# PlantandFoodResearch/MCHap

Measured on AMD Instinct MI355X. Metric: loci/sec (whole node) for 1000-step MCMC, tetraploid 8-SNV loci, 1/2/4/8 GPUs, higher is better.
Workload: dtype f64; 1 GPU; 10000 synthetic tetraploid loci per GPU, 8 SNVs, 200 reads, 1000 MCMC steps x 2 chains, burn 500, posterior summary (BASELINE.json configs[1]); 4 passes in flight on separate HIP streams, each with its own device buffers; loci_per_gpu=10000, ploidy=4, snvs=8, reads=200, mcmc_steps=1000, chains=2, burn=500, llk_cache=True, passes_in_flight=4, hw_queues=4, world_size=1, devices=1

## Files before the change

mchap_amd/csrc/denovo_kernel.hpp:

```cpp
#pragma once
#include <hip/hip_runtime.h>
#include <math.h>
#include <stdint.h>

#include "../../include/mchap_hip.h"
#include "philox.hpp"

namespace mchap {

constexpr int WAVE = 64;
constexpr uint32_t SLOT_INIT = 0xFFFFu;

static __constant__ double c_ln[260];
static __constant__ double c_ln_inv[260];

struct DenovoParams {
  const mchap_unit *units;
  const double *reads;
  const int64_t *counts;
  const int8_t *n_alleles;
  const int8_t *initial;
  uint64_t *trace;
  double *llks;
  int8_t *fixed;
// ... 42 lines not shown
  if (nb < M + 4) nb = M + 4;
  L.buf = o; o += 8 * nb;
  L.optin = o; o += 4 * K * K;
  L.sub = o; o += align8(2 * K * M);
  L.hetrow = o; o += align8(2 * M);
  L.shift = o; o += align8(M);
  L.nal = o; o += align8(M);
  L.total = align8(o);
  return L;
}

__host__ __device__ inline int allele_bits(int A) { return A <= 2 ? 1 : (A <= 4 ? 2 : 3); }

template <int CTRL>
__device__ __forceinline__ double wave_dpp_f64(double v) {
  const long long b = __double_as_longlong(v);
  const int lo = __builtin_amdgcn_update_dpp(0, (int)(unsigned)b, CTRL, 0xf, 0xf, false);
  const int hi = __builtin_amdgcn_update_dpp(0, (int)(unsigned)((unsigned long long)b >> 32), CTRL, 0xf, 0xf, false);
  return __longlong_as_double((long long)(((unsigned long long)(unsigned)hi << 32) | (unsigned)lo));
}
__device__ __forceinline__ double wave_sum(double v) {
#ifdef MCHAP_PLAIN_BUTTERFLY
#pragma unroll
  for (int o = 32; o >= 1; o >>= 1) v += __shfl_xor(v, o, WAVE);
#else
  v += __shfl_xor(v, 32, WAVE);
  v += __shfl_xor(v, 16, WAVE);
  v += wave_dpp_f64<0x128>(v);
  v += wave_dpp_f64<0x124>(v);
  v += wave_dpp_f64<0x122>(v);
  v += wave_dpp_f64<0x121>(v);
#endif
  return v;
}
static __global__ void wave_sum_kernel(const double *x, double *out) {
  const double s = wave_sum(x[(size_t)blockIdx.x * WAVE + threadIdx.x]);
  const bool same = __ballot(__double_as_longlong(s) == __double_as_longlong(__shfl(s, 0, WAVE))) == ~0ull;
  if (threadIdx.x == 0) out[blockIdx.x] = same ? s : __longlong_as_double(0x7ff8dead00000000ll);
}
__device__ __forceinline__ int wave_sum_i(int v) {
#pragma unroll
  for (int o = 32; o >= 1; o >>= 1) v += __shfl_xor(v, o, WAVE);
  return v;
}

__device__ __forceinline__ uint32_t nib(uint32_t p, int h) { return (p >> (4 * h)) & 15u; }
__device__ __forceinline__ uint32_t nib_set(uint32_t p, int h, uint32_t v) {
  return (p & ~(15u << (4 * h))) | (v << (4 * h));
}
__device__ __forceinline__ uint32_t nib(uint64_t p, int h) { return (uint32_t)(p >> (4 * h)) & 15u; }
__device__ __forceinline__ uint64_t nib_set(uint64_t p, int h, uint32_t v) {
  return (p & ~(15ull << (4 * h))) | ((uint64_t)v << (4 * h));
}

__device__ __forceinline__ double add_log_prob(double x, double y) {
  if (x == -INFINITY && y == -INFINITY) return -INFINITY;
  if (x > y) return x + log1p(exp(y - x));
  return y + log1p(exp(x - y));
}

__device__ __forceinline__ int choose_from(const double *p, int n, double u) {
  double c = 0.0;
  for (int i = 0; i < n; i++) {
    c += p[i];
    if (c > u) return i;
  }
// ... 783 lines not shown
```

mchap_amd/csrc/denovo_spec_kernel.hpp:

```cpp
#pragma once
#include <type_traits>

#include "denovo_simt_kernel.hpp"

#ifdef MCHAP_MASK_PADDING
#define MCHAP_PAD_LANE(x) (x)
#else
#define MCHAP_PAD_LANE(x) true
#endif
#ifndef MCHAP_COOP_UNR
#define MCHAP_COOP_UNR 2
#endif
#ifndef MCHAP_SPEC_TB
#define MCHAP_SPEC_TB 4
#endif
#ifndef MCHAP_SPEC_LOW
#define MCHAP_SPEC_LOW 8
#endif
#ifndef MCHAP_SPEC_CG
#define MCHAP_SPEC_CG 4
#endif
#ifndef MCHAP_SPEC_VAR
#define MCHAP_SPEC_VAR 0
#endif
#define MCHAP_SPEC_SBS (MCHAP_SPEC_VAR == 1)
#define MCHAP_SPEC_DEEP (MCHAP_SPEC_VAR == 2)
#ifndef MCHAP_SPEC_WIN0
#define MCHAP_SPEC_WIN0 4
#endif
#ifndef MCHAP_SPEC_WIN_MIN
#define MCHAP_SPEC_WIN_MIN 2
#endif
#ifndef MCHAP_REUSE_MAXK
#define MCHAP_REUSE_MAXK 8
#endif
#ifndef MCHAP_CODED_UNR
#define MCHAP_CODED_UNR 16
#endif

namespace mchap {

constexpr int SPEC_MAX_IV = 64;
constexpr int SPEC_TB = MCHAP_SPEC_TB;
constexpr int SPEC_LN = 72;
constexpr int SPEC_DRAWS_MAX = 384;
__host__ __device__ inline int spec_draws(int K, int Mmax) {
  int d = 2 * K * Mmax - 1;
  if (d < 3 * Mmax + 2) d = 3 * Mmax + 2;
  d = (d + 1) & ~1;
  return d < SPEC_DRAWS_MAX ? d : SPEC_DRAWS_MAX;
}

#define LDSP(T) __attribute__((address_space(3))) T *
#define GLBP(T) __attribute__((address_space(1))) T *
template <class T>
__device__ __forceinline__ LDSP(T) lds_cast(void *p) {
  return (LDSP(T))p;
}

// ... 26 lines not shown
  LDSP(double) optp;
  LDSP(double) optl;
  LDSP(double) ln;
  LDSP(double) lninv;
  LDSP(uint32_t) ivse;
  LDSP(uint32_t) ivlin;
  LDSP(uint32_t) ivlout;
  LDSP(uint32_t) ivno;
  LDSP(uint16_t) cols;
  LDSP(uint16_t) permtab;
  LDSP(uint8_t) shift;
  LDSP(uint8_t) nal;
  LDSP(uint8_t) ktab;
  LDSP(uint8_t) ordtab;
  LDSP(uint16_t) nreads;
  LDSP(uint16_t) ndict;
  LDSP(double) dict;
  LDSP(uint64_t) gptr;
  LDSP(double) gval;
  LDSP(uint32_t) gstream;
  LDSP(uint64_t) bw;
  LDSP(double) bpc;
  LDSP(uint64_t) bpt;
  LDSP(uint64_t) gbt;
  LDSP(const uint8_t) sct;
  LDSP(uint64_t) tbuf;
  LDSP(uint64_t) lc;
  uint32_t lc_mask;
  uint32_t cache_mask;
  int key_words;
  bool cache_on;
  uint64_t epoch = 0ull;
  bool reuse_on;
  bool cut_off = false;
  LDSP(const uint8_t) lds_ct;
  LDSP(const double) lds_cw;
  int crow;
  LDSP(uint64_t) draws;
  LDSP(double) memo_tot;
  LDSP(double) bdist;
  int memo_stride;
  int ndraws;
  LDSP(unsigned char) cx_lds;
  LDSP(double) cx_val;
  uint64_t *cx_base = nullptr;
  int cx_n = 0;
};

__host__ __device__ inline int spec_memo_entries(int Mmax) { return Mmax * (Mmax + 1) / 2; }
__host__ __device__ inline int spec_memo_index(int start, int stop) { return stop * (stop - 1) / 2 + start; }
__host__ __device__ inline size_t spec_memo_bytes(int Mmax, int T, int G) {
  const size_t per_group = (size_t)2 * spec_memo_entries(Mmax) * 8;
  if (T != 1 || per_group > 16 * 1024) return 0;
  return per_group * (64 / G);
}

constexpr int SPEC_LC_ENTRIES = 256;
#ifndef MCHAP_LC_GEN
#define MCHAP_LC_GEN 48
#endif
constexpr uint32_t SPEC_LC_SECOND_LEVEL_GEN = MCHAP_LC_GEN;
__host__ __device__ inline size_t spec_lc_bytes(int entries = SPEC_LC_ENTRIES) { return (size_t)16 * entries + 16; }
__host__ __device__ inline bool spec_ctx_in_bpc(int K, int Mmax, int Amax, int max_reads) {
  return K >= 3 && max_reads <= 64 && Mmax * Amax <= 24 * (K - 2) && 16 * K * Mmax <= 3 * 64 * 8 && 12 * 64 + 4 * 8 <= 3 * 64 * 8;
}
__host__ __device__ inline int spec_lc_entries(int bp_cache) { return (bp_cache & 2) ? ((bp_cache & 4) ? SPEC_LC_ENTRIES / 2 : SPEC_LC_ENTRIES) : 0; }
// ... 536 lines not shown
__device__ __forceinline__ void spec_hap_prod(LDSP(double) dict, const PairRows rows, int p0, int Mh, typename TabPtr<LT>::u8 ct,
                                              int crow, double (&prod)[RPL]) {
  constexpr int UNR = 8;
  constexpr int GB = 2;
#pragma unroll
  for (int i = 0; i < RPL; i++) prod[i] = 1.0;
  for (int j0 = 0; j0 < Mh; j0 += UNR) {
    CT cd[UNR];
#pragma unroll
    for (int u = 0; u < UNR; u++) {
      const int p = __builtin_amdgcn_readfirstlane(p0 + min(j0 + u, Mh - 1));
      const int row = p < WAVE ? __builtin_amdgcn_readlane(rows.r0, p & (WAVE - 1))
                               : (p < 2 * WAVE ? __builtin_amdgcn_readlane(rows.r1, p & (WAVE - 1)) : __builtin_amdgcn_readlane(rows.r2, p & (WAVE - 1)));
      cd[u] = TabPtr<LT>::template ld<CT>(ct + (size_t)row * crow);
    }
#pragma unroll
    for (int u0 = 0; u0 < UNR; u0 += GB) {
      if (j0 + u0 < Mh) {
        double f[GB][RPL];
#pragma unroll
        for (int u = 0; u < GB; u++)
#pragma unroll
          for (int i = 0; i < RPL; i++) f[u][i] = dict[((uint32_t)cd[u0 + u] >> (8 * i)) & 255u];
#pragma unroll
        for (int u = 0; u < GB; u++) {
          const bool on = j0 + u0 + u < Mh;
#pragma unroll
          for (int i = 0; i < RPL; i++) prod[i] *= on ? f[u][i] : 1.0;
        }
      }
    }
  }
}
template <int KT, bool IN_LDS>
struct BaseProducts;
template <int KT>
struct BaseProducts<KT, false> {
  double v[KT][4];
  __device__ __forceinline__ double get(int h, int i, int) const { return v[h][i]; }
  __device__ __forceinline__ void set(int h, int i, int, double x) { v[h][i] = x; }
};
template <int KT>
struct BaseProducts<KT, true> {
  LDSP(double) p;
  __device__ __forceinline__ double get(int h, int i, int lane) const { return p[(h * 4 + i) * WAVE + lane]; }
  __device__ __forceinline__ void set(int h, int i, int lane, double x) { p[(h * 4 + i) * WAVE + lane] = x; }
};
template <int KT>
struct BaseProductsG {
  GLBP(double) p;
  int rpad, cb;
  __device__ __forceinline__ double get(int h, int i, int lane) const { return p[(size_t)h * rpad + (cb + i) * WAVE + lane]; }
  __device__ __forceinline__ void set(int h, int i, int lane, double x) { p[(size_t)h * rpad + (cb + i) * WAVE + lane] = x; }
};
template <int KT, int RPL, class CT, bool LT = false, class BP>
__device__ __forceinline__ double spec_coop_reuse(const SpecLds &S, int src, int sg, int mmax, int Mh, uint32_t amask,
                                                  typename TabPtr<LT>::u8 ct, typename TabPtr<LT>::f64 cw, int crow, int lane,
                                                  const BP &bp, bool use_base, bool grouped) {
  LDSP(double) dict = S.dict + (size_t)sg * DICT_MAX;
  const double invK = 1.0 / (double)KT;
  const PairRows rows = spec_pair_rows<KT>(S.pw, WAVE, src, S, sg, mmax, Mh, amask, lane);
  double acc[RPL];
#pragma unroll
  for (int i = 0; i < RPL; i++) acc[i] = 0.0;
#pragma unroll
  for (int h = 0; h < KT; h++) {
    const uint64_t a = S.pw[(size_t)h * WAVE + src], b = S.bw[(size_t)sg * KT + h];
    const bool same = use_base && __builtin_amdgcn_readfirstlane((int)(a == b)) != 0;
    double ph[RPL];
    if (same) {
#pragma unroll
      for (int i = 0; i < RPL; i++) ph[i] = bp.get(h, i, lane);
    } else {
      spec_hap_prod<RPL, CT, LT>(dict, rows, h * Mh, Mh, ct, crow, ph);
    }
#pragma unroll
    for (int i = 0; i < RPL; i++) acc[i] += ph[i] * invK;
  }
  double wv[RPL];
#pragma unroll
  for (int i = 0; i < RPL; i++) wv[i] = cw[WAVE * i];
  return read_log_sum<RPL>(acc, wv, grouped);
}
template <int KT, int RPL, class CT, bool LT = false>
__device__ __forceinline__ double spec_coop_reuse_g(const SpecLds &S, int src, int sg, int mmax, int Mh, uint32_t amask,
                                                    typename TabPtr<LT>::u8 ct, typename TabPtr<LT>::f64 cw, int crow, int lane,
                                                    const BaseProductsG<KT> &bg, bool grouped) {
  double bpv[KT][RPL];
#pragma unroll
  for (int h = 0; h < KT; h++)
#pragma unroll
    for (int i = 0; i < RPL; i++) bpv[h][i] = bg.get(h, i, lane);
  LDSP(double) dict = S.dict + (size_t)sg * DICT_MAX;
  const double invK = 1.0 / (double)KT;
  const PairRows rows = spec_pair_rows<KT>(S.pw, WAVE, src, S, sg, mmax, Mh, amask, lane);
  double acc[RPL];
#pragma unroll
  for (int i = 0; i < RPL; i++) acc[i] = 0.0;
#pragma unroll
  for (int h = 0; h < KT; h++) {
    const uint64_t a = S.pw[(size_t)h * WAVE + src], b = S.bw[(size_t)sg * KT + h];
    const bool same = __builtin_amdgcn_readfirstlane((int)(a == b)) != 0;
    double ph[RPL];
    if (same) {
#pragma unroll
      for (int i = 0; i < RPL; i++) ph[i] = bpv[h][i];
    } else {
      spec_hap_prod<RPL, CT, LT>(dict, rows, h * Mh, Mh, ct, crow, ph);
    }
#pragma unroll
    for (int i = 0; i < RPL; i++) acc[i] += ph[i] * invK;
  }
  double wv[RPL];
#pragma unroll
  for (int i = 0; i < RPL; i++) wv[i] = cw[WAVE * i];
  return read_log_sum<RPL>(acc, wv, grouped);
}
template <int KT, int RPL, class CT, bool LT = false, class BP>
__device__ __forceinline__ void spec_base_products(const SpecLds &S, int sg, int mmax, int Mh, uint32_t amask,
                                                   typename TabPtr<LT>::u8 ct, int crow, int lane, BP &bp) {
  LDSP(double) dict = S.dict + (size_t)sg * DICT_MAX;
  const PairRows rows = spec_pair_rows<KT>(S.bw + (size_t)sg * KT, 1, 0, S, sg, mmax, Mh, amask, lane);
#pragma unroll
  for (int h = 0; h < KT; h++) {
    double ph[RPL];
    spec_hap_prod<RPL, CT, LT>(dict, rows, h * Mh, Mh, ct, crow, ph);
#pragma unroll
    for (int i = 0; i < RPL; i++) bp.set(h, i, lane, ph[i]);
  }
}
template <int KT, int RPL, class CT, bool LT = false, class BP>
__device__ __forceinline__ void spec_base_products_of(const SpecLds &S, const PairRows rows, int sg, int h, int Mh,
                                                      typename TabPtr<LT>::u8 ct, int crow, int lane, BP &bp) {
  LDSP(double) dict = S.dict + (size_t)sg * DICT_MAX;
  double ph[RPL];
  spec_hap_prod<RPL, CT, LT>(dict, rows, h * Mh, Mh, ct, crow, ph);
#pragma unroll
  for (int i = 0; i < RPL; i++) bp.set(h, i, lane, ph[i]);
}

template <int KT>
__device__ __forceinline__ unsigned long long spec_same_request(LDSP(uint64_t) pwbuf, unsigned long long reqs, int src, int lane) {
  if ((reqs & (reqs - 1ull)) == 0ull) return reqs;
  bool eq = ((reqs >> lane) & 1ull) != 0ull;
#pragma unroll
  for (int h = 0; h < KT; h++) eq = eq & (pwbuf[(size_t)h * WAVE + lane] == pwbuf[(size_t)h * WAVE + src]);
  return __ballot(eq);
}

template <int KT, int G, bool LT = false, bool DEDUP = true>
__device__ __forceinline__ double spec_coop_all(unsigned long long todo, LDSP(uint64_t) pwbuf, LDSP(uint8_t) shift_tab,
                                                LDSP(uint16_t) cols_tab, LDSP(uint16_t) nreads_tab, LDSP(uint16_t) ndict_tab,
                                                LDSP(double) dict_tab, LDSP(uint64_t) gptr_tab, LDSP(uint64_t) bw_tab,
                                                bool reuse, int crow, int mmax, int Mh_lane, uint32_t amask_lane, int rpad,
                                                int lane, LDSP(const uint8_t) lds_ct = nullptr, LDSP(const double) lds_cw = nullptr,
                                                LDSP(double) bpc = nullptr, LDSP(uint64_t) bpt = nullptr,
                                                LDSP(const uint8_t) sct = nullptr, LDSP(uint64_t) gbt = nullptr) {
  SpecLds S;
  S.pw = pwbuf;
  S.shift = shift_tab;
  S.cols = cols_tab;
  S.dict = dict_tab;
  S.bw = bw_tab;
  const int nch_batch = rpad / WAVE;
  double val = 0.0;
  while (todo) {
    const int sg = (__ffsll((long long)todo) - 1) / G;
    const unsigned long long gmask = G == 64 ? ~0ull : (((1ull << (G & 63)) - 1ull) << (sg * (G & 63)));
    unsigned long long reqs = todo & gmask;
    todo &= ~gmask;
    const int first = __ffsll((long long)reqs) - 1;
    const int Mh = __builtin_amdgcn_readfirstlane(__shfl(Mh_lane, first, WAVE));
    const uint32_t amask = (uint32_t)__builtin_amdgcn_readfirstlane(__shfl((int)amask_lane, first, WAVE));
    LDSP(uint64_t) gp = gptr_tab + sg * GP_N;
    GLBP(const double) rt = (GLBP(const double))(uintptr_t)gp[GP_RT] + lane;
    typename TabPtr<LT>::f64 cw;
    if constexpr (LT) cw = lds_cw + lane;
    else cw = (GLBP(const double))(uintptr_t)gp[GP_CW] + lane;
    const int nrd = (int)nreads_tab[sg];
    const bool grouped = nd_w01(ndict_tab[sg]);
    const int nch = max(1, min(nch_batch, (nrd + WAVE - 1) / WAVE));
    const int cstride = crow / WAVE;
    if (MCHAP_REUSE_MAXK >= KT && nd_count(ndict_tab[sg]) != 0 && KT * Mh <= (MCHAP_SPEC_DEEP ? 3 : 2) * WAVE) {
      const int nb0 = nch < 4 ? nch : 4;
      typename TabPtr<LT>::u8 ct;
      if constexpr (LT) ct = lds_ct + (size_t)lane * cstride;
      else ct = (GLBP(const uint8_t))(uintptr_t)gp[GP_CT] + (size_t)lane * cstride;
      constexpr bool BPL = (G == 64) && !LT;
      bool cached = false;
      if (BPL && bpc != nullptr) {
// ... 303 lines not shown
              double acc[4] = {0.0, 0.0, 0.0, 0.0};
#pragma unroll
              for (int h = 0; h < KT; h++) {
                const uint64_t wa = pwbuf[(size_t)h * WAVE + my_src], wb = bw_tab[(size_t)sg * KT + h];
                double ph[4];
                if (wa == wb) {
#pragma unroll
                  for (int k = 0; k < 4; k++) ph[k] = k < RK ? bpc[(h * 4) * WAVE + r + 16 * k] : 0.0;
                } else {
                  hap_products(wa, ph);
                }
#pragma unroll
                for (int k = 0; k < 4; k++) acc[k] += ph[k] * invK;
              }
#pragma unroll
              for (int k = 0; k < 4; k++)
                if (k < RK) v[k] = read_log(acc[k]) * cwr[k];
            }
            const double a0 = RK > 2 ? v[0] + v[2] : v[0];
            const double a1 = RK > 3 ? v[1] + v[3] : v[1];
            double sv = RK > 1 ? a0 + a1 : a0;
#pragma unroll
            for (int o = 8; o >= 1; o >>= 1) sv += __shfl_xor(sv, o, WAVE);
#pragma unroll
            for (int k = 0; k < 4; k++) {
              const double vk = __shfl(sv, 16 * k, WAVE);
              if (k < nq && ((dupm[k] >> lane) & 1ull)) val = vk;
            }
          }
          continue;
        }
      }
#endif
      while (reqs) {
        const int src = __ffsll((long long)reqs) - 1;
        const unsigned long long dups = (DEDUP ? spec_same_request<KT>(pwbuf, reqs, src, lane) : (1ull << src));
        reqs &= ~dups;
        double s = 0.0;
        if (nb0 == 1) s += spec_coop_reuse<KT, 1, uint8_t, LT>(S, src, sg, mmax, Mh, amask, ct, cw, crow, lane, bp, use_base, grouped);
        else if (nb0 == 2) s += spec_coop_reuse<KT, 2, uint16_t, LT>(S, src, sg, mmax, Mh, amask, ct, cw, crow, lane, bp, use_base, grouped);
        else if (nb0 == 3) s += spec_coop_reuse<KT, 3, uint32_t, LT>(S, src, sg, mmax, Mh, amask, ct, cw, crow, lane, bp, use_base, grouped);
        else s += spec_coop_reuse<KT, 4, uint32_t, LT>(S, src, sg, mmax, Mh, amask, ct, cw, crow, lane, bp, use_base, grouped);
        for (int cb = 4; cb < nch; cb += 4) {
          const int rem = nch - cb;
          typename TabPtr<LT>::f64 cwb = cw + cb * WAVE;
          if (deep) {
            BaseProductsG<KT> bg;
            bg.p = gbp;
            bg.rpad = rpad;
            bg.cb = cb;
            if (rem >= 4) s += spec_coop_reuse_g<KT, 4, uint32_t, LT>(S, src, sg, mmax, Mh, amask, ct + cb, cwb, crow, lane, bg, grouped);
            else if (rem == 3) s += spec_coop_reuse_g<KT, 3, uint32_t, LT>(S, src, sg, mmax, Mh, amask, ct + cb, cwb, crow, lane, bg, grouped);
            else if (rem == 2) s += spec_coop_reuse_g<KT, 2, uint16_t, LT>(S, src, sg, mmax, Mh, amask, ct + cb, cwb, crow, lane, bg, grouped);
            else s += spec_coop_reuse_g<KT, 1, uint8_t, LT>(S, src, sg, mmax, Mh, amask, ct + cb, cwb, crow, lane, bg, grouped);
          } else {
            if (rem >= 4) s += spec_coop_coded<KT, 4, uint32_t, LT>(S, src, sg, mmax, Mh, amask, ct + cb, cwb, crow, lane, grouped);
            else if (rem == 3) s += spec_coop_coded<KT, 3, uint32_t, LT>(S, src, sg, mmax, Mh, amask, ct + cb, cwb, crow, lane, grouped);
            else if (rem == 2) s += spec_coop_coded<KT, 2, uint16_t, LT>(S, src, sg, mmax, Mh, amask, ct + cb, cwb, crow, lane, grouped);
            else s += spec_coop_coded<KT, 1, uint8_t, LT>(S, src, sg, mmax, Mh, amask, ct + cb, cwb, crow, lane, grouped);
          }
        }
        s = wave_sum(s);
        if ((dups >> lane) & 1ull) val = s;
      }
    } else {
      while (reqs) {
        const int src = __ffsll((long long)reqs) - 1;
        const unsigned long long dups = (DEDUP ? spec_same_request<KT>(pwbuf, reqs, src, lane) : (1ull << src));
        reqs &= ~dups;
        double s = 0.0;
        const bool coded = nd_count(ndict_tab[sg]) != 0;
        typename TabPtr<LT>::u8 ct;
        if constexpr (LT) ct = lds_ct + (size_t)lane * cstride;
        else ct = (GLBP(const uint8_t))(uintptr_t)gp[GP_CT] + (size_t)lane * cstride;
        GLBP(const double) cwg = (GLBP(const double))(uintptr_t)gp[GP_CW] + lane;
        for (int cb = 0; cb < nch; cb += 4) {
          const int rem = nch - cb;
          typename TabPtr<LT>::f64 cwb = cw + cb * WAVE;
          if (coded) {
            if (rem >= 4) s += spec_coop_coded<KT, 4, uint32_t, LT>(S, src, sg, mmax, Mh, amask, ct + cb, cwb, crow, lane, grouped);
            else if (rem == 3) s += spec_coop_coded<KT, 3, uint32_t, LT>(S, src, sg, mmax, Mh, amask, ct + cb, cwb, crow, lane, grouped);
            else if (rem == 2) s += spec_coop_coded<KT, 2, uint16_t, LT>(S, src, sg, mmax, Mh, amask, ct + cb, cwb, crow, lane, grouped);
            else s += spec_coop_coded<KT, 1, uint8_t, LT>(S, src, sg, mmax, Mh, amask, ct + cb, cwb, crow, lane, grouped);
          } else {
            GLBP(const double) rtb = rt + cb * WAVE;
            GLBP(const double) cwgb = cwg + cb * WAVE;
            if (rem >= 4) s += spec_coop_body<KT, 4>(S, src, sg, mmax, Mh, amask, rtb, cwgb, rpad, lane, nrd - cb * WAVE, grouped);
            else if (rem == 3) s += spec_coop_body<KT, 3>(S, src, sg, mmax, Mh, amask, rtb, cwgb, rpad, lane, nrd - cb * WAVE, grouped);
            else if (rem == 2) s += spec_coop_body<KT, 2>(S, src, sg, mmax, Mh, amask, rtb, cwgb, rpad, lane, nrd - cb * WAVE, grouped);
            else s += spec_coop_body<KT, 1>(S, src, sg, mmax, Mh, amask, rtb, cwgb, rpad, lane, nrd - cb * WAVE, grouped);
          }
        }
        s = wave_sum(s);
        if ((dups >> lane) & 1ull) val = s;
      }
    }
  }
  return val;
}

struct SpecKeepAll {
  __device__ __forceinline__ bool operator()(bool miss, double) const { return miss; }
};
template <int KT, int G, bool LT = false, class Filter = SpecKeepAll, bool DEDUP = true>
__device__ __forceinline__ double spec_eval(bool need, const GWords<KT> pw, const Grp<KT> &c, const SpecLds &S, int mmax,
                                            int rpad, int lane, Filter filt = Filter()) {
  double val = 0.0;
  if (c.flat) {
    val = c.llk;
    need = false;
  }
  bool miss = need;
  uint64_t tag = 0;
  ulonglong2 *slot = nullptr;
  GSUB_T0();
  const bool wide = C_KEYBITS(c) * KT > 63;
  uint64_t *kslot = nullptr;
  LDSP(uint64_t) lslot = S.lc;
  bool promote = false;
  if (need && S.cache_on) {
    tag = tag_of<KT>(pw, C_KEYBITS(c), S.epoch);
    const uint64_t key = tag >> 1;
    uint32_t hsh = (uint32_t)key ^ ((uint32_t)(key >> 32) * 0x9E3779B1u);
    hsh ^= hsh >> 16;
    hsh *= 0x7FEB352Du;
    hsh ^= hsh >> 15;
    hsh *= 0x846CA68Bu;
    hsh ^= hsh >> 16;
    const size_t set_i = (size_t)((hsh >> 12) & S.cache_mask);
    ulonglong2 *set = reinterpret_cast<ulonglong2 *>((uintptr_t)S.gptr[(lane / G) * GP_N + GP_CACHE]) + 8 * set_i;
    int way = (int)((hsh >> 24) & 7u);
    if (S.lc_mask != 0u && !wide) {
      LDSP(uint64_t) le = S.lc + 2 * (size_t)((hsh >> 3) & S.lc_mask);
      const uint64_t t = le[0], v = le[1];
      if (t == tag) {
        val = __longlong_as_double((long long)v);
        miss = false;
// ... 33 lines not shown
          miss = true;
          way = hit_way;
        }
      }
      kslot = kset + (size_t)way * S.key_words;
    }
    }
    slot = set + way;
  }
  if (wave_any(promote)) {
    if (promote) lslot[0] = tag;
    lds_sync();
    if (promote && lslot[0] == tag) lslot[1] = (uint64_t)__double_as_longlong(val);
    lds_sync();
  }
  miss = filt(miss, val);
  STAT_ADD(0, need);
  STAT_ADD(1, miss);
  STAT_ADD(2, true);
  unsigned long long todo = __ballot(miss);
  GSUB(c, 9);
  if (todo) {
    GCOUNT(c, 11, __popcll(todo));
    if (miss) {
#pragma unroll
      for (int h = 0; h < KT; h++) S.pw[(size_t)h * WAVE + lane] = pw.w[h];
    }
    if (S.reuse_on && lane % G == 0) {
      const GWords<KT> cg = c.g;
#pragma unroll
      for (int h = 0; h < KT; h++) S.bw[(size_t)(lane / G) * KT + h] = cg.w[h];
    }
    lds_sync();
    const double v = spec_coop_all<KT, G, LT, DEDUP>(todo, S.pw, S.shift, S.cols, S.nreads, S.ndict, S.dict, S.gptr, S.bw, S.reuse_on, S.crow, mmax, c.Mh, C_AMASK(c), rpad, lane, S.lds_ct, S.lds_cw, S.bpc, S.bpt, S.sct, S.gbt);
    if (miss) val = v;
    bool writer = miss && slot != nullptr;
    if (wave_any(writer && wide)) {
      unsigned long long pend = __ballot(writer);
      bool mine = false;
      while (pend) {
        const int l = __ffsll((long long)pend) - 1;
        const unsigned long long sl = __shfl((unsigned long long)(uintptr_t)slot, l, WAVE);
        const unsigned long long same = __ballot(writer && (unsigned long long)(uintptr_t)slot == sl);
        if (lane == l) mine = true;
        pend &= ~same;
      }
      writer = mine;
    }
    if (writer) {
      if (wide) {
#pragma unroll
        for (int h = 0; h < KT; h++) kslot[h] = pw.w[h];
      }
      *slot = make_ulonglong2(tag, (unsigned long long)__double_as_longlong(val));
    }
    if (S.lc_mask != 0u && !wide) {
      if (writer) lslot[0] = tag;
      lds_sync();
      if (writer && lslot[0] == tag) lslot[1] = (uint64_t)__double_as_longlong(val);
    }
    lds_sync();
    GSUB(c, 10);
  }
  return val;
}

#ifndef MCHAP_SPEC_WPE
// ... 214 lines not shown
        u = staged ? draw_double(dtab[n - 1 + p]) : stream_double(ld_stream(S, gi), ctr0 + (uint64_t)(n - 1) + (uint64_t)p);
      }
      const uint64_t wh = sel_word<KT>(c.g, h);
      const int current = (int)((wh >> sh) & C_AMASK(c));
      const double lhapcount = S.ln[copies_of<KT>(c.g, wh)];
      const double ln_opt = S.ln[n_alleles - 1];
      double sum = 0.0;
      bool dropped = false;
#pragma unroll 1
      for (int o = 0; o < amax - 1; o++) {
        const bool prop = act && o < n_alleles - 1;
        const int i = o + (o >= current ? 1 : 0);
        GWords<KT> pw = c.g;
        const uint64_t nw = (wh & ~((uint64_t)C_AMASK(c) << sh)) | ((uint64_t)i << sh);
        set_word<KT>(pw, h, nw);
        auto known_mover_cuts = [&](bool miss, double v) -> bool {
          if (!cut_on) return miss;
          bool mv = false;
          if (prop && !miss) {
            double lprior_ratio = 0.0;
            if (!isnan(C_INB(S, gi))) lprior_ratio = prior_of<KT>(pt, C_INB(S, gi), dosage_words<KT>(pw)) - lprior;
            const double lproposal_ratio = S.ln[copies_of<KT>(pw, nw)] - lhapcount;
            const double mh = ((v - c.llk) + lprior_ratio) * temp + lproposal_ratio;
            const double pr = exp(fmin(0.0, mh) - ln_opt);
            const double stay = 1.0 - (0.0 + pr);
            mv = current == 0 ? !(0.0 + stay > u) : (0.0 + pr > u);
          }
          const uint64_t mm = grp_ballot<G>(mv, gi);
          const bool keep = miss && (mm == 0ull || gl < __ffsll((long long)mm) - 1);
          dropped = dropped || (miss && !keep);
          return keep;
        };
        GT0(t_ev);
        const double llk_i = spec_eval<KT, G, LT, decltype(known_mover_cuts), G != 64>(prop, pw, c, S, mmax, rpad, lane, known_mover_cuts);
        GT1(c, 16, t_ev);
        if (prop) {
          double lprior_ratio = 0.0;
          if (!isnan(C_INB(S, gi))) lprior_ratio = prior_of<KT>(pt, C_INB(S, gi), dosage_words<KT>(pw)) - lprior;
          const double lproposal_ratio = S.ln[copies_of<KT>(pw, nw)] - lhapcount;
          const double mh = ((llk_i - c.llk) + lprior_ratio) * temp + lproposal_ratio;
          const double pr = exp(fmin(0.0, mh) - ln_opt);
          if constexpr (CTX && G == 64) {
            if (cx && !dropped) {
              const int e_ = permtab[p];
              const int ei = (e_ >> 8) * Mh + (e_ & 255);
              CXP_PR(S)[ei] = pr;
              CXP_LLK(S, nmax)[ei] = llk_i;
              uint64_t *sp = S.cx_base + (size_t)(CXP_ST(S)[CX_CUR] - 1u) * spec_ctx_words(KT, mmax) + SPEC_CTX_HDR;
              ctx_st(sp + ei, pr);
              ctx_st(sp + nmax + ei, llk_i);
            }
          }
          S.optp[o * WAVE + lane] = pr;
          S.optl[o * WAVE + lane] = llk_i;
          sum += pr;
        }
      }
      bool changed = false;
      uint64_t neww = 0;
      double newllk = 0.0;
      if (act && !dropped) {
        const double stay = 1.0 - sum;
        double cacc = 0.0;
        int choice = -1;
        double cl = c.llk;
        for (int i = 0; i < n_alleles && choice < 0; i++) {
          double pi = stay, li = c.llk;
// ... 622 lines not shown
  long long q = my_slot;
  const long long n_chains = (long long)P.n_units * Cn;
  Grp<KT> c;
  c.alive = q < n_chains;
  bool listed = false;
  if constexpr (PIPE) {
    listed = q < n_list;
    c.alive = listed;
    if (listed && P.pipe_list) q = P.pipe_list[q];
    if (!listed) q = 0;
  }
  const bool resume = PIPE && (P.pipe_mode & PIPE_RESUME);
  int base = 0;
  const int u = c.alive ? (int)(q / Cn) : 0;
  const int chain = c.alive ? (int)(q % Cn) : 0;
  const mchap_unit U = D.units[u];
  const int32_t *mi = P.meta_i + (size_t)u * meta_i_stride(P.max_pos);
  const double *mf = P.meta_f + (size_t)u * meta_f_stride(P.max_ploidy, P.max_pos, P.max_allele);
  if (c.alive && mi[META_I_STATUS] != MCHAP_UNIT_OK) c.alive = false;
  const int A = U.max_allele;
  c.Mh = c.alive ? mi[META_I_MH] : 1;
  c.bits = allele_bits(A);
  c.flat = c.alive && mi[META_I_FLAT] != 0 && !(P.flags & 128);
  if (gl == 0) {
    S.gval[gi * GV_N + GV_INB] = U.inbreeding;
    S.gval[gi * GV_N + GV_MLO] = 0.0;
    S.gval[gi * GV_N + GV_MHI] = 0.0;
    S.gstream[gi * 4 + 0] = (uint32_t)D.seed;
    S.gstream[gi * 4 + 1] = (uint32_t)(D.seed >> 32) ^ (uint32_t)(U.stream_id >> 32);
    S.gstream[gi * 4 + 2] = ((uint32_t)chain << 16) | 0u;
    S.gstream[gi * 4 + 3] = (uint32_t)U.stream_id;
  }
  S.reuse_on = !(P.flags & 8);
  S.cut_off = (P.flags & 262144) != 0;
  S.lds_ct = nullptr;
  S.lds_cw = nullptr;
  S.crow = WAVE * P.cstride;
  S.cache_on = D.cache_slots > 0 && !fillonly;
  S.cache_mask = S.cache_on ? (uint32_t)(D.cache_slots / 8) - 1u : 0u;
  S.epoch = P.cache_epoch;
  S.key_words = D.cache_key_words;
  if (gl == 0) {
    LDSP(uint64_t) gp = S.gptr + gi * GP_N;
    gp[GP_RT] = (uint64_t)(uintptr_t)(P.rt + (size_t)u * P.max_ma * rpad);
    gp[GP_CW] = (uint64_t)(uintptr_t)(P.cntw + (size_t)u * rpad);
    gp[GP_CT] = (uint64_t)(uintptr_t)(P.codes + (size_t)u * P.max_ma * WAVE * P.cstride);
    const size_t qc = (size_t)q * (size_t)(PIPE ? 1 : D.n_temps) + (size_t)tw;
    gp[GP_CACHE] = S.cache_on ? (uint64_t)(uintptr_t)(reinterpret_cast<ulonglong2 *>(D.cache) + qc * (size_t)D.cache_slots) : 0ull;
    gp[GP_CKEYS] = (S.cache_on && D.cache_keys) ? (uint64_t)(uintptr_t)(D.cache_keys + qc * (size_t)D.cache_slots * D.cache_key_words) : 0ull;
    gp[GP_TRACE] = (uint64_t)(uintptr_t)(D.trace + U.trace_off + (size_t)chain * D.steps * KT);
    gp[GP_LLK] = (uint64_t)(uintptr_t)(D.llks + U.llk_off + (size_t)chain * D.steps);
    gp[GP_GBP] = P.gbp ? (uint64_t)(uintptr_t)(P.gbp + ((size_t)q * (PIPE ? 1 : D.n_temps) + tw) * P.max_ploidy * rpad) : 0ull;
  }
  c.ctr = 0;
  c.doff = 0;
  c.dcount = 0;
  c.llk = 0.0;
  c.memo_on = (T == 1) && !(P.flags & 1);
  c.mvalid = false;
  c.mwin = MCHAP_SPEC_WIN0;
  c.fill_part = fillonly ? my_part : 0;
  c.fill_parts = fillonly ? parts_eff : 1;
  c.gen = 1;
  c.memo_gen = 1;
  if constexpr (CTX && G == 64 && PIPE) {
    if (S.cx_n > 0 && c.alive) S.cx_base = P.ctx + (size_t)q * (size_t)P.ctx_n * (size_t)spec_ctx_words(KT, mmax);
// ... 386 lines not shown
```

mchap_amd/csrc/mchap_hip.hip:

```cpp
#include <hip/hip_runtime.h>

#include <cmath>
#include <cstdarg>
#include <cstdio>
#include <cstdlib>
#include <cstring>
#include <algorithm>
#include <atomic>
#include <mutex>
#include <vector>

#include "../../include/mchap_hip.h"
#include "denovo_kernel.hpp"
#include "denovo_simt_kernel.hpp"
#include "denovo_spec_kernel.hpp"
#include "denovo_fillw_kernel.hpp"
#ifdef MCHAP_TEST_KERNELS
#include "denovo_fill_kernel.hpp"
#include "denovo_lane_kernel.hpp"
#endif
#include "exact_kernel.hpp"
#include "call_mcmc_kernel.hpp"
#include "posterior_kernel.hpp"

// ... 1032 lines not shown
      P.cache = reinterpret_cast<uint64_t *>(ws + cv.cache);
      P.cache_slots = slots;
      uint64_t epoch = 0;
      if ((pl.kind == SAMPLER_PIPE || pl.kind == SAMPLER_SPEC) && !(T.flags & (64 | 65536)) &&
          B.max_ploidy * mchap::allele_bits(B.max_allele) * B.max_pos <= 32) {
        epoch = cfg->cache_epoch > 0 ? (uint64_t)cfg->cache_epoch : g_cache_epoch.fetch_add(1) + 1;
        if (epoch >= (1ull << 31) - 1) epoch = 0;
      }
      SP.cache_epoch = epoch << 33;
      if (!epoch)
        HIP_TRY(hipMemsetAsync(ws + cv.cache, 0, (size_t)n_units * cfg->chains * (pl.kind == SAMPLER_SPEC ? cfg->n_temps : 1) * slots * 16, stream));
      if (cv.key_words) {
        P.cache_keys = reinterpret_cast<uint64_t *>(ws + cv.ckeys);
        P.cache_key_words = cv.key_words;
      }
    }
    SP.rt = reinterpret_cast<double *>(ws + cv.rt);
    SP.cntw = reinterpret_cast<double *>(ws + cv.cntw);
    SP.codes = ws + cv.codes;
    SP.dict = reinterpret_cast<double *>(ws + cv.dict);
    SP.gbp = (cv.has_gbp && !(T.flags & 512)) ? reinterpret_cast<double *>(ws + cv.gbp) : nullptr;
    SP.meta_i = reinterpret_cast<int32_t *>(ws + cv.meta_i);
    SP.meta_f = reinterpret_cast<double *>(ws + cv.meta_f);
    SP.lane_state = ws + cv.lane_state;
    SP.lane_memo = ws + cv.lane_memo;
    SP.pipe_state = ws + cv.pipe_state;
    SP.pipe_memo = reinterpret_cast<double *>(ws + cv.pipe_memo);
    SP.n_units = n_units;
    SP.max_pos = B.max_pos;
    SP.max_allele = B.max_allele;
    SP.max_ploidy = B.max_ploidy;
    SP.max_ma = B.max_ma;
    SP.cstride = code_stride(rpl);
    SP.flags = T.flags & (63 | 128 | 2048 | 4096 | 262144 | (1 << 20));
    SP.max_ugens_pad = (B.max_ugens + 8) & ~7;
    const size_t lds_dict = (size_t)mchap::DICT_HASH * (8 + 2) + 64;
    size_t lds_prep = (size_t)B.max_ma * rpad * 8 + (size_t)SP.max_ugens_pad * 8 + lds_dict;
    SP.prep_rows_off = 0;
    if (lds_prep > 160 * 1024 || (size_t)B.max_ma * rpad * 8 > T.prep_lds_limit) {
      lds_prep = (size_t)SP.max_ugens_pad * 8 + lds_dict;
      lds_prep = (lds_prep + 15) & ~(size_t)15;
      SP.prep_rows_off = (int)lds_prep;
      lds_prep += (size_t)B.max_allele * rpad * 8;
      SP.flags |= mchap::SIMT_FLAG_PREP_GLOBAL;
    }
    const size_t lds_simt = mchap::simt_lds_bytes(B.max_ploidy, B.max_pos, cfg->n_temps, pl.wide ? 16 : 8);
    SP.word_bits = pl.wide ? 128 : 64;
    if (lds_prep > 160 * 1024 || lds_simt > 160 * 1024)
      return fail(MCHAP_ERR_LIMIT, "a unit needs %zu / %zu bytes of LDS (> 160 KiB)", lds_prep, lds_simt);
    auto prepare = [&](const mchap::SimtParams &Q, int n, hipStream_t st) {
      switch (rpl) {
        case 1: return launch_prepare<1>(Q, n, lds_prep, st);
        case 2: return launch_prepare<2>(Q, n, lds_prep, st);
        case 3: return launch_prepare<3>(Q, n, lds_prep, st);
        case 4: return launch_prepare<4>(Q, n, lds_prep, st);
        case 5: return launch_prepare<5>(Q, n, lds_prep, st);
        case 6: return launch_prepare<6>(Q, n, lds_prep, st);
        case 7: return launch_prepare<7>(Q, n, lds_prep, st);
        case 8: return launch_prepare<8>(Q, n, lds_prep, st);
        case 12: return launch_prepare<12>(Q, n, lds_prep, st);
        case 16: return launch_prepare<16>(Q, n, lds_prep, st);
        case 24: return launch_prepare<24>(Q, n, lds_prep, st);
        case 32: return launch_prepare<32>(Q, n, lds_prep, st);
        case 48: return launch_prepare<48>(Q, n, lds_prep, st);
        default: return launch_prepare<64>(Q, n, lds_prep, st);
      }
    };
// ... 213 lines not shown
```

mchap_amd/csrc/read_log.hpp:

```cpp
#pragma once
#include <hip/hip_runtime.h>

namespace mchap {

__device__ __forceinline__ double read_log_core(double m, int e, double x) {
  const bool small = m < 0.70710678118654752440;
  m = small ? m * 2.0 : m;
  e = small ? e - 1 : e;
  const double f = m - 1.0;
  const double d = 2.0 + f;
  double r = __builtin_amdgcn_rcp(d);
  r = fma(fma(-d, r, 1.0), r, r);
  r = fma(fma(-d, r, 1.0), r, r);
  double s = f * r;
  s = fma(fma(-d, s, f), r, s);
  const double z = s * s, w = z * z;
  const double t1 = w * fma(w, fma(w, 1.531383769920937332e-01, 2.222219843214978396e-01), 3.999999999940941908e-01);
  const double t2 = z * fma(w, fma(w, fma(w, 1.479819860511658591e-01, 1.818357216161805012e-01), 2.857142874366239149e-01),
                            6.666666666666735130e-01);
  const double R = t2 + t1;
  const double hfsq = 0.5 * f * f;
  const double k = (double)e;
  double v = k * 6.93147180369123816490e-01 - ((hfsq - (s * (hfsq + R) + k * 1.90821492927058770002e-10)) - f);
  v = x == 0.0 ? -INFINITY : v;
// ... 3 lines not shown

__device__ __forceinline__ double read_log(double x) {
  return read_log_core(__builtin_amdgcn_frexp_mant(x), __builtin_amdgcn_frexp_exp(x), x);
}

template <int N>
__device__ __forceinline__ double read_log_product(const double (&x)[N]) {
  static_assert(N >= 1 && N <= 4, "groups of at most four reads: the product of four mantissas stays above 2^-4");
  if constexpr (N == 1) return read_log(x[0]);
  double m = __builtin_amdgcn_frexp_mant(x[0]);
  int e = __builtin_amdgcn_frexp_exp(x[0]);
#pragma unroll
  for (int i = 1; i < N; i++) {
    m *= __builtin_amdgcn_frexp_mant(x[i]);
    e += __builtin_amdgcn_frexp_exp(x[i]);
  }
  return read_log_core(__builtin_amdgcn_frexp_mant(m), e + __builtin_amdgcn_frexp_exp(m), m);
}
template <int N>
__device__ __forceinline__ double read_log_sum(const double (&x)[N], const double (&w)[N], bool grouped) {
  if (grouped) {
    double y[N];
#pragma unroll
    for (int i = 0; i < N; i++) y[i] = w[i] != 0.0 ? x[i] : 1.0;
    return read_log_product<N>(y);
  }
  double s = 0.0;
#pragma unroll
  for (int i = 0; i < N; i++) s += read_log(x[i]) * w[i];
  return s;
}

template <int N>
__device__ __forceinline__ double read_log_sum_chunks(const double (&x)[N], const double (&w)[N], bool grouped) {
  if constexpr (N <= 4) {
    return read_log_sum<N>(x, w, grouped);
  } else {
    static_assert(N % 4 == 0, "chunks in fours");
    double s = 0.0;
    if (grouped) {
#pragma unroll
      for (int g = 0; g < N / 4; g++) {
        double y[4];
#pragma unroll
        for (int i = 0; i < 4; i++) y[i] = w[4 * g + i] != 0.0 ? x[4 * g + i] : 1.0;
        s += read_log_product<4>(y);
      }
    } else {
#pragma unroll
      for (int i = 0; i < N; i++) s += read_log(x[i]) * w[i];
    }
    return s;
  }
}

static __global__ void read_log_kernel(const double *x, long long n, double *out) {
  for (long long i = (long long)blockIdx.x * blockDim.x + threadIdx.x; i < n; i += (long long)gridDim.x * blockDim.x) out[i] = read_log(x[i]);
}

}
```

Measured before the change: 1.112 million loci/s.

## Evaluate two single-haplotype-change likelihood requests together in cooperative spec path

```diff
diff --git a/mchap_amd/csrc/denovo_kernel.hpp b/mchap_amd/csrc/denovo_kernel.hpp
--- a/mchap_amd/csrc/denovo_kernel.hpp
+++ b/mchap_amd/csrc/denovo_kernel.hpp
@@ -98,6 +98,29 @@
   v += wave_dpp_f64<0x121>(v);
 #endif
   return v;
+}
+__device__ __forceinline__ void wave_sum2(double &a, double &b) {
+#ifdef MCHAP_PLAIN_BUTTERFLY
+#pragma unroll
+  for (int o = 32; o >= 1; o >>= 1) {
+    const double ta = __shfl_xor(a, o, WAVE), tb = __shfl_xor(b, o, WAVE);
+    a += ta;
+    b += tb;
+  }
+#else
+  double ta = __shfl_xor(a, 32, WAVE), tb = __shfl_xor(b, 32, WAVE);
+  a += ta, b += tb;
+  ta = __shfl_xor(a, 16, WAVE), tb = __shfl_xor(b, 16, WAVE);
+  a += ta, b += tb;
+  ta = wave_dpp_f64<0x128>(a), tb = wave_dpp_f64<0x128>(b);
+  a += ta, b += tb;
+  ta = wave_dpp_f64<0x124>(a), tb = wave_dpp_f64<0x124>(b);
+  a += ta, b += tb;
+  ta = wave_dpp_f64<0x122>(a), tb = wave_dpp_f64<0x122>(b);
+  a += ta, b += tb;
+  ta = wave_dpp_f64<0x121>(a), tb = wave_dpp_f64<0x121>(b);
+  a += ta, b += tb;
+#endif
 }
 static __global__ void wave_sum_kernel(const double *x, double *out) {
   const double s = wave_sum(x[(size_t)blockIdx.x * WAVE + threadIdx.x]);
diff --git a/mchap_amd/csrc/denovo_spec_kernel.hpp b/mchap_amd/csrc/denovo_spec_kernel.hpp
--- a/mchap_amd/csrc/denovo_spec_kernel.hpp
+++ b/mchap_amd/csrc/denovo_spec_kernel.hpp
@@ -25,6 +25,16 @@
 #endif
 #define MCHAP_SPEC_SBS (MCHAP_SPEC_VAR == 1)
 #define MCHAP_SPEC_DEEP (MCHAP_SPEC_VAR == 2)
+#ifndef MCHAP_SPEC_PAIR_MAXK
+#define MCHAP_SPEC_PAIR_MAXK 4
+#endif
+#ifndef MCHAP_SPEC_PAIR
+#if defined(SPEC_PIPE) && MCHAP_SPEC_VAR == 0
+#define MCHAP_SPEC_PAIR 1
+#else
+#define MCHAP_SPEC_PAIR 0
+#endif
+#endif
 #ifndef MCHAP_SPEC_WIN0
 #define MCHAP_SPEC_WIN0 4
 #endif
@@ -117,6 +127,7 @@
   bool cache_on;
   uint64_t epoch = 0ull;
   bool reuse_on;
+  bool pair_on;
   bool cut_off = false;
   LDSP(const uint8_t) lds_ct;
   LDSP(const double) lds_cw;
@@ -719,6 +730,50 @@
     }
   }
 }
+template <int RPL, class CT>
+__device__ __forceinline__ void spec_hap_prod2(LDSP(double) dict, const PairRows ra, const PairRows rb, int pa, int pb, int Mh,
+                                               GLBP(const uint8_t) ct, int crow, double (&proda)[RPL], double (&prodb)[RPL]) {
+  constexpr int UNR = 8;
+  constexpr int GB = 1;
+#pragma unroll
+  for (int i = 0; i < RPL; i++) proda[i] = 1.0, prodb[i] = 1.0;
+  for (int j0 = 0; j0 < Mh; j0 += UNR) {
+    CT ca[UNR], cb[UNR];
+#pragma unroll
+    for (int u = 0; u < UNR; u++) {
+      const int jj = min(j0 + u, Mh - 1);
+      const int p = __builtin_amdgcn_readfirstlane(pa + jj), q = __builtin_amdgcn_readfirstlane(pb + jj);
+      const int rowa = p < WAVE ? __builtin_amdgcn_readlane(ra.r0, p & (WAVE - 1))
+                                : (p < 2 * WAVE ? __builtin_amdgcn_readlane(ra.r1, p & (WAVE - 1)) : __builtin_amdgcn_readlane(ra.r2, p & (WAVE - 1)));
+      const int rowb = q < WAVE ? __builtin_amdgcn_readlane(rb.r0, q & (WAVE - 1))
+                                : (q < 2 * WAVE ? __builtin_amdgcn_readlane(rb.r1, q & (WAVE - 1)) : __builtin_amdgcn_readlane(rb.r2, q & (WAVE - 1)));
+      ca[u] = TabPtr<false>::template ld<CT>(ct + (size_t)rowa * crow);
+      cb[u] = TabPtr<false>::template ld<CT>(ct + (size_t)rowb * crow);
+    }
+#pragma unroll
+    for (int u0 = 0; u0 < UNR; u0 += GB) {
+      if (j0 + u0 < Mh) {
+        double fa[GB][RPL], fb[GB][RPL];
+#pragma unroll
+        for (int u = 0; u < GB; u++)
+#pragma unroll
+          for (int i = 0; i < RPL; i++) {
+            fa[u][i] = dict[((uint32_t)ca[u0 + u] >> (8 * i)) & 255u];
+            fb[u][i] = dict[((uint32_t)cb[u0 + u] >> (8 * i)) & 255u];
+          }
+#pragma unroll
+        for (int u = 0; u < GB; u++) {
+          const bool on = j0 + u0 + u < Mh;
+#pragma unroll
+          for (int i = 0; i < RPL; i++) {
+            proda[i] *= on ? fa[u][i] : 1.0;
+            prodb[i] *= on ? fb[u][i] : 1.0;
+          }
+        }
+      }
+    }
+  }
+}
 template <int KT, bool IN_LDS>
 struct BaseProducts;
 template <int KT>
@@ -769,6 +824,33 @@
   for (int i = 0; i < RPL; i++) wv[i] = cw[WAVE * i];
   return read_log_sum<RPL>(acc, wv, grouped);
 }
+template <int KT, int RPL, class CT, class BP>
+__device__ __forceinline__ void spec_coop_pair(const SpecLds &S, int srca, int srcb, int ha, int hb, int sg, int mmax, int Mh,
+                                               uint32_t amask, GLBP(const uint8_t) ct, GLBP(const double) cw, int crow, int lane,
+                                               const BP &bp, bool grouped, double &sa, double &sb) {
+  LDSP(double) dict = S.dict + (size_t)sg * DICT_MAX;
+  const double invK = 1.0 / (double)KT;
+  const PairRows ra = spec_pair_rows<KT>(S.pw, WAVE, srca, S, sg, mmax, Mh, amask, lane);
+  const PairRows rb = spec_pair_rows<KT>(S.pw, WAVE, srcb, S, sg, mmax, Mh, amask, lane);
+  double pa[RPL], pb[RPL];
+  spec_hap_prod2<RPL, CT>(dict, ra, rb, ha * Mh, hb * Mh, Mh, ct, crow, pa, pb);
+  double wv[RPL];
+#pragma unroll
+  for (int i = 0; i < RPL; i++) wv[i] = cw[WAVE * i];
+  double acca[RPL], accb[RPL];
+#pragma unroll
+  for (int i = 0; i < RPL; i++) acca[i] = 0.0, accb[i] = 0.0;
+#pragma unroll
+  for (int h = 0; h < KT; h++) {
+#pragma unroll
+    for (int i = 0; i < RPL; i++) {
+      const double b = bp.get(h, i, lane);
+      acca[i] += (h == ha ? pa[i] : b) * invK;
+      accb[i] += (h == hb ? pb[i] : b) * invK;
+    }
+  }
+  read_log_sum2<RPL>(acca, accb, wv, grouped, sa, sb);
+}
 template <int KT, int RPL, class CT, bool LT = false>
 __device__ __forceinline__ double spec_coop_reuse_g(const SpecLds &S, int src, int sg, int mmax, int Mh, uint32_t amask,
                                                     typename TabPtr<LT>::u8 ct, typename TabPtr<LT>::f64 cw, int crow, int lane,
@@ -835,14 +917,15 @@
   return __ballot(eq);
 }
 
-template <int KT, int G, bool LT = false, bool DEDUP = true>
+template <int KT, int G, bool LT = false, bool DEDUP = true, bool PAIR = false>
 __device__ __forceinline__ double spec_coop_all(unsigned long long todo, LDSP(uint64_t) pwbuf, LDSP(uint8_t) shift_tab,
                                                 LDSP(uint16_t) cols_tab, LDSP(uint16_t) nreads_tab, LDSP(uint16_t) ndict_tab,
                                                 LDSP(double) dict_tab, LDSP(uint64_t) gptr_tab, LDSP(uint64_t) bw_tab,
                                                 bool reuse, int crow, int mmax, int Mh_lane, uint32_t amask_lane, int rpad,
                                                 int lane, LDSP(const uint8_t) lds_ct = nullptr, LDSP(const double) lds_cw = nullptr,
                                                 LDSP(double) bpc = nullptr, LDSP(uint64_t) bpt = nullptr,
-                                                LDSP(const uint8_t) sct = nullptr, LDSP(uint64_t) gbt = nullptr) {
+                                                LDSP(const uint8_t) sct = nullptr, LDSP(uint64_t) gbt = nullptr,
+                                                bool pair_on = false) {
   SpecLds S;
   S.pw = pwbuf;
   S.shift = shift_tab;
@@ -1212,10 +1295,42 @@
         }
       }
 #endif
+      const bool pair_ok = PAIR && BPL && pair_on && use_base && nch > 1 && nch <= 4;
       while (reqs) {
         const int src = __ffsll((long long)reqs) - 1;
         const unsigned long long dups = (DEDUP ? spec_same_request<KT>(pwbuf, reqs, src, lane) : (1ull << src));
         reqs &= ~dups;
+        if constexpr (PAIR && BPL) {
+          if (pair_ok && reqs) {
+            const int srcb = __ffsll((long long)reqs) - 1;
+            int ha = 0, hb = 0, na = 0, nb = 0;
+#pragma unroll
+            for (int h = 0; h < KT; h++) {
+              const uint64_t wb = bw_tab[(size_t)sg * KT + h];
+              const bool da = pwbuf[(size_t)h * WAVE + src] != wb, db = pwbuf[(size_t)h * WAVE + srcb] != wb;
+              ha = da ? h : ha;
+              hb = db ? h : hb;
+              na += da ? 1 : 0;
+              nb += db ? 1 : 0;
+            }
+            if (__builtin_amdgcn_readfirstlane((int)(na == 1 && nb == 1)) != 0) {
+              ha = __builtin_amdgcn_readfirstlane(ha);
+              hb = __builtin_amdgcn_readfirstlane(hb);
+              const unsigned long long dupsb = (DEDUP ? spec_same_request<KT>(pwbuf, reqs, srcb, lane) : (1ull << srcb));
+              reqs &= ~dupsb;
+              STAT_WAVE(22, 1);
+              double sa = 0.0, sb = 0.0;
+              if (nb0 == 2) spec_coop_pair<KT, 2, uint16_t>(S, src, srcb, ha, hb, sg, mmax, Mh, amask, ct, cw, crow, lane, bp, grouped, sa, sb);
+              else if (nb0 == 3) spec_coop_pair<KT, 3, uint32_t>(S, src, srcb, ha, hb, sg, mmax, Mh, amask, ct, cw, crow, lane, bp, grouped, sa, sb);
+              else spec_coop_pair<KT, 4, uint32_t>(S, src, srcb, ha, hb, sg, mmax, Mh, amask, ct, cw, crow, lane, bp, grouped, sa, sb);
+              wave_sum2(sa, sb);
+              if ((dups >> lane) & 1ull) val = sa;
+              if ((dupsb >> lane) & 1ull) val = sb;
+              continue;
+            }
+          }
+        }
+        STAT_WAVE(23, 1);
         double s = 0.0;
         if (nb0 == 1) s += spec_coop_reuse<KT, 1, uint8_t, LT>(S, src, sg, mmax, Mh, amask, ct, cw, crow, lane, bp, use_base, grouped);
         else if (nb0 == 2) s += spec_coop_reuse<KT, 2, uint16_t, LT>(S, src, sg, mmax, Mh, amask, ct, cw, crow, lane, bp, use_base, grouped);
@@ -1282,7 +1397,7 @@
 struct SpecKeepAll {
   __device__ __forceinline__ bool operator()(bool miss, double) const { return miss; }
 };
-template <int KT, int G, bool LT = false, class Filter = SpecKeepAll, bool DEDUP = true>
+template <int KT, int G, bool LT = false, class Filter = SpecKeepAll, bool DEDUP = true, bool PAIR = false>
 __device__ __forceinline__ double spec_eval(bool need, const GWords<KT> pw, const Grp<KT> &c, const SpecLds &S, int mmax,
                                             int rpad, int lane, Filter filt = Filter()) {
   double val = 0.0;
@@ -1382,7 +1497,7 @@
       for (int h = 0; h < KT; h++) S.bw[(size_t)(lane / G) * KT + h] = cg.w[h];
     }
     lds_sync();
-    const double v = spec_coop_all<KT, G, LT, DEDUP>(todo, S.pw, S.shift, S.cols, S.nreads, S.ndict, S.dict, S.gptr, S.bw, S.reuse_on, S.crow, mmax, c.Mh, C_AMASK(c), rpad, lane, S.lds_ct, S.lds_cw, S.bpc, S.bpt, S.sct, S.gbt);
+    const double v = spec_coop_all<KT, G, LT, DEDUP, PAIR>(todo, S.pw, S.shift, S.cols, S.nreads, S.ndict, S.dict, S.gptr, S.bw, S.reuse_on, S.crow, mmax, c.Mh, C_AMASK(c), rpad, lane, S.lds_ct, S.lds_cw, S.bpc, S.bpt, S.sct, S.gbt, S.pair_on);
     if (miss) val = v;
     bool writer = miss && slot != nullptr;
     if (wave_any(writer && wide)) {
@@ -1663,7 +1778,7 @@
           return keep;
         };
         GT0(t_ev);
-        const double llk_i = spec_eval<KT, G, LT, decltype(known_mover_cuts), G != 64>(prop, pw, c, S, mmax, rpad, lane, known_mover_cuts);
+        const double llk_i = spec_eval<KT, G, LT, decltype(known_mover_cuts), G != 64, MCHAP_SPEC_PAIR && !CTX && KT <= MCHAP_SPEC_PAIR_MAXK>(prop, pw, c, S, mmax, rpad, lane, known_mover_cuts);
         GT1(c, 16, t_ev);
         if (prop) {
           double lprior_ratio = 0.0;
@@ -2352,6 +2467,7 @@
     S.gstream[gi * 4 + 3] = (uint32_t)U.stream_id;
   }
   S.reuse_on = !(P.flags & 8);
+  S.pair_on = !(P.flags & 2097152);
   S.cut_off = (P.flags & 262144) != 0;
   S.lds_ct = nullptr;
   S.lds_cw = nullptr;
diff --git a/mchap_amd/csrc/mchap_hip.hip b/mchap_amd/csrc/mchap_hip.hip
--- a/mchap_amd/csrc/mchap_hip.hip
+++ b/mchap_amd/csrc/mchap_hip.hip
@@ -1088,7 +1088,7 @@
     SP.max_ploidy = B.max_ploidy;
     SP.max_ma = B.max_ma;
     SP.cstride = code_stride(rpl);
-    SP.flags = T.flags & (63 | 128 | 2048 | 4096 | 262144 | (1 << 20));
+    SP.flags = T.flags & (63 | 128 | 2048 | 4096 | 262144 | (1 << 20) | (1 << 21));
     SP.max_ugens_pad = (B.max_ugens + 8) & ~7;
     const size_t lds_dict = (size_t)mchap::DICT_HASH * (8 + 2) + 64;
     size_t lds_prep = (size_t)B.max_ma * rpad * 8 + (size_t)SP.max_ugens_pad * 8 + lds_dict;
diff --git a/mchap_amd/csrc/read_log.hpp b/mchap_amd/csrc/read_log.hpp
--- a/mchap_amd/csrc/read_log.hpp
+++ b/mchap_amd/csrc/read_log.hpp
@@ -59,6 +59,31 @@
 }
 
 template <int N>
+__device__ __forceinline__ void read_log_sum2(const double (&xa)[N], const double (&xb)[N], const double (&w)[N], bool grouped,
+                                              double &ra, double &rb) {
+  if (grouped) {
+    double ya[N], yb[N];
+#pragma unroll
+    for (int i = 0; i < N; i++) {
+      ya[i] = w[i] != 0.0 ? xa[i] : 1.0;
+      yb[i] = w[i] != 0.0 ? xb[i] : 1.0;
+    }
+    ra = read_log_product<N>(ya);
+    rb = read_log_product<N>(yb);
+    return;
+  }
+  double sa = 0.0, sb = 0.0;
+#pragma unroll
+  for (int i = 0; i < N; i++) {
+    const double la = read_log(xa[i]), lb = read_log(xb[i]);
+    sa += la * w[i];
+    sb += lb * w[i];
+  }
+  ra = sa;
+  rb = sb;
+}
+
+template <int N>
 __device__ __forceinline__ double read_log_sum_chunks(const double (&x)[N], const double (&w)[N], bool grouped) {
   if constexpr (N <= 4) {
     return read_log_sum<N>(x, w, grouped);
```

Result: faster. 1.164 million loci/s (median of 5 runs) (+4.7%).
